# lucidrains/progen

Hardware: AMD Instinct MI355X
Metric: train tokens/sec (whole node) (higher is better)
Workload: dtype bf16; 1 GPU; model=ProGen-1.2B, global_batch=64, seq_len=1024, parallelism=dp1

## Files before the change

progen_amd/models/progen.py:

```python

from __future__ import annotations

import math
from typing import Any, Dict, Optional

import torch
import torch.nn as nn

from ..config import ProGenConfig
from ..ops import functional as OF
from ..ops import reference as R


def _haiku_linear_init_(weight: torch.Tensor, bias: Optional[torch.Tensor],
                        generator: Optional[torch.Generator] = None) -> None:
    fan_in = weight.shape[1]
    std = 1.0 / math.sqrt(fan_in)
    with torch.no_grad():
        weight.normal_(0.0, std, generator=generator).clamp_(-2 * std, 2 * std)
        if bias is not None:
            bias.zero_()


class Linear(nn.Linear):

    def reset_parameters(self) -> None:
        _haiku_linear_init_(self.weight, self.bias)

    def forward(self, x: torch.Tensor) -> torch.Tensor:
        from ..ops import fp8
        if fp8.fp8_eligible(x, self.weight):
            return fp8.fp8_linear(x, self.weight, self.bias)
        from ..ops.overlap import overlap_linear
        return overlap_linear(x, self.weight, self.bias)


class LocalAttention(nn.Module):

    def __init__(self, cfg: ProGenConfig):
        super().__init__()
        self.heads = cfg.heads
        self.window_size = cfg.window_size
        self.shift_tokens = cfg.shift_tokens
        inner = cfg.inner_dim
        self.norm_weight = nn.Parameter(torch.ones(cfg.dim))
        self.to_qkv = Linear(cfg.dim, inner * 3, bias=False)
        self.to_out = Linear(inner, cfg.dim, bias=True)

    def forward(self, x: torch.Tensor, sin: torch.Tensor, cos: torch.Tensor) -> torch.Tensor:
        x = OF.ln_shift(x, self.norm_weight, shift=self.shift_tokens)
        return self.inner(x, sin, cos)

    def inner(self, y: torch.Tensor, sin: torch.Tensor, cos: torch.Tensor) -> torch.Tensor:
        qkv = self.to_qkv(y)
        out = OF.local_attention(qkv, sin, cos, self.heads, self.window_size)
        return self.to_out(out)


class SGU(nn.Module):

    def __init__(self, dim: int, dim_out: int, seq_len: int, eps: float = 1e-3):
        super().__init__()
        self.seq_len = seq_len
        self.norm_weight = nn.Parameter(torch.ones(dim // 2))
        init_scale = eps / seq_len
        self.spatial_weights = nn.Parameter(
            torch.empty(seq_len, seq_len).uniform_(-init_scale, init_scale))
        self.spatial_biases = nn.Parameter(torch.ones(seq_len, 1))
        self.proj_out = Linear(dim // 2, dim_out, bias=True)

    def forward(self, x: torch.Tensor) -> torch.Tensor:
# ... 9 lines not shown
        assert not (glu and spatial_gate), \
            "glu and sgu cannot be turned on at the same time"
        hidden = cfg.dim * cfg.ff_mult * (2 if glu else 1)
        self.glu = glu
        self.shift_tokens = cfg.shift_tokens
        self.norm_weight = nn.Parameter(torch.ones(cfg.dim))
        self.proj_in = Linear(cfg.dim, hidden, bias=True)
        self.sgu = SGU(hidden, hidden // 2, cfg.seq_len) if spatial_gate else None
        out_in = hidden // 2 if (glu or spatial_gate) else hidden
        self.proj_out = Linear(out_in, cfg.dim, bias=True)

    def forward(self, x: torch.Tensor) -> torch.Tensor:
        x = OF.ln_shift(x, self.norm_weight, shift=self.shift_tokens)
        return self.inner(x)

    def inner(self, x: torch.Tensor) -> torch.Tensor:
        x = self.proj_in(x)
        if self.glu:
            x = OF.glu_gelu(x)
        else:
            x = OF.gelu(x)
        if self.sgu is not None:
            x = self.sgu(x)
        return self.proj_out(x)


class ProGenBase(nn.Module):

    def __init__(self, cfg: ProGenConfig):
        super().__init__()
        self.cfg = cfg
        self.embed = nn.Embedding(cfg.num_tokens, cfg.dim)
        with torch.no_grad():
            std = 1.0 / math.sqrt(cfg.num_tokens)
            self.embed.weight.normal_(0.0, std).clamp_(-2 * std, 2 * std)

        layers = []
        for i in range(cfg.depth):
            use_gmlp = (cfg.depth - i) <= cfg.global_mlp_depth
# ... 11 lines not shown
        self.register_buffer("rotary_sin", sin, persistent=False)
        self.register_buffer("rotary_cos", cos, persistent=False)

    def forward(self, x: torch.Tensor) -> torch.Tensor:
        if x.dim() == 1:
            x = x.unsqueeze(0)
        n = x.shape[1]
        if self.rotary_sin.dtype != torch.float32:
            sin, cos = R.fixed_pos_embedding(self.cfg.seq_len,
                                             self.cfg.dim_head,
                                             device=self.rotary_sin.device)
            self.rotary_sin, self.rotary_cos = sin, cos
        sin = self.rotary_sin[:n]
        cos = self.rotary_cos[:n]
        h = self.embed(x.long())
        r = None
        for attn, ff in self.layers:
            y, h = OF.ln_shift_res(h, r, attn.norm_weight,
                                   shift=attn.shift_tokens)
            a = attn.inner(y, sin, cos)
            y, h = OF.ln_shift_res(h, a, ff.norm_weight,
                                   shift=ff.shift_tokens)
            r = ff.inner(y)
        y, _ = OF.ln_shift_res(h, r, self.final_norm_weight, shift=False)
        return self.to_logits(y)

    def num_params(self) -> int:
        return sum(p.numel() for p in self.parameters())



class TransformedProGen:

    def __init__(self, cfg: ProGenConfig, module: Optional[ProGenBase] = None):
        self.cfg = cfg
        self.module = module if module is not None else ProGenBase(cfg)

    @staticmethod
    def _seed_everything(rng) -> None:
# ... 37 lines not shown
```

progen_amd/ops/functional.py:

```python

from __future__ import annotations

import torch
import torch.nn.functional as F

from . import dispatch, reference



class _LnShiftFn(torch.autograd.Function):
    @staticmethod
    def forward(ctx, x, weight, shift: bool, eps: float):
        C = dispatch.ext()
        y, mean, rstd = C.ln_shift_fwd(x, weight, bool(shift), float(eps))
        ctx.save_for_backward(x, weight, mean, rstd)
        ctx.shift = bool(shift)
        return y

    @staticmethod
    def backward(ctx, dy):
        x, weight, mean, rstd = ctx.saved_tensors
        C = dispatch.ext()
        dx, dweight = C.ln_shift_bwd(dy.contiguous(), x, weight, mean, rstd, ctx.shift)
        return dx, dweight, None, None


def ln_shift(x: torch.Tensor, weight: torch.Tensor, shift: bool = True,
             eps: float = 1e-5) -> torch.Tensor:
    if dispatch.use_hip(x, "ln"):
        return _LnShiftFn.apply(x, weight, shift, eps)
    return reference.ln_shift(x, weight, shift, eps)


class _LnShiftResFn(torch.autograd.Function):

    @staticmethod
    def forward(ctx, x, res, weight, shift: bool, eps: float):
        C = dispatch.ext()
        y, s, mean, rstd = C.ln_shift_res_fwd(x, res, weight, bool(shift),
                                              float(eps))
        ctx.save_for_backward(s, weight, mean, rstd)
        ctx.shift = bool(shift)
        ctx.set_materialize_grads(False)
        return y, s

    @staticmethod
    def backward(ctx, dy, ds):
        s, weight, mean, rstd = ctx.saved_tensors
        C = dispatch.ext()
        ds = ds.contiguous() if ds is not None else None
        dx, dweight = C.ln_shift_res_bwd(dy.contiguous(), ds, s, weight,
                                         mean, rstd, ctx.shift)
        return dx, dx, dweight, None, None


def ln_shift_res(x: torch.Tensor, res, weight: torch.Tensor,
                 shift: bool = True, eps: float = 1e-5):
    if dispatch.use_hip(x, "ln"):
        if res is None:
            return _LnShiftFn.apply(x, weight, shift, eps), x
        return _LnShiftResFn.apply(x, res.contiguous(), weight, shift, eps)
    s = x if res is None else x + res
    return reference.ln_shift(s, weight, shift, eps), s



class _LocalAttnFn(torch.autograd.Function):
    @staticmethod
    def forward(ctx, qkv, sin, cos, heads: int, window_size: int, halo):
        C = dispatch.ext()
        qkv_rot = C.rope_qkv(qkv.contiguous(), sin, cos)
        out, lse = C.attn_fwd(qkv_rot, int(heads), int(window_size),
                              halo=halo)
        ctx.save_for_backward(qkv_rot, sin, cos, out, lse,
                              *([halo] if halo is not None else []))
        ctx.heads = int(heads)
# ... 12 lines not shown
        dhalo = res[1].to(dout.dtype) if ctx.has_halo else None
        return dqkv, None, None, None, None, dhalo


def local_attention(qkv: torch.Tensor, sin: torch.Tensor, cos: torch.Tensor,
                    heads: int, window_size: int,
                    halo: torch.Tensor = None) -> torch.Tensor:
    if dispatch.use_hip(qkv, "attn"):
        return _LocalAttnFn.apply(qkv, sin, cos, heads, window_size, halo)
    assert halo is None, "halo is a kernel-path (GPU) feature"
    return reference.local_attention(qkv, sin, cos, heads, window_size)



class _GluGeluFn(torch.autograd.Function):
    @staticmethod
    def forward(ctx, h):
        C = dispatch.ext()
        y = C.glu_fwd(h)
        ctx.save_for_backward(h)
        return y

    @staticmethod
    def backward(ctx, dy):
        (h,) = ctx.saved_tensors
        C = dispatch.ext()
        return C.glu_bwd(dy.contiguous(), h)


def glu_gelu(h: torch.Tensor) -> torch.Tensor:
    if dispatch.use_hip(h, "glu"):
        return _GluGeluFn.apply(h)
    return reference.glu_gelu(h)


class _GeluFn(torch.autograd.Function):
    @staticmethod
    def forward(ctx, h):
        C = dispatch.ext()
        y = C.gelu_fwd(h)
        ctx.save_for_backward(h)
        return y

    @staticmethod
    def backward(ctx, dy):
        (h,) = ctx.saved_tensors
        C = dispatch.ext()
# ... 264 lines not shown
```

progen_amd/ops/hip/bindings.cpp:

```cpp

#include <torch/extension.h>

#include "checks.h"
#include "kernels.h"

using namespace chk;


static std::vector<at::Tensor> ln_shift_fwd_impl(const char* op,
                                                 const at::Tensor& x,
                                                 const at::Tensor* res,
                                                 const at::Tensor& g,
                                                 bool shift, double eps) {
  const bool bf = dtype_bf16_or_fp32(op, ARG(x));
  dtype_same(op, ARG(g), ARG(x));
  if (res) dtype_same(op, Arg{"res", *res}, ARG(x));
  contiguous_rank(op, ARG(x), 3);
  const int64_t B = x.size(0), N = x.size(1), D = x.size(2);
  if (res) contiguous_shape(op, Arg{"res", *res}, x.sizes());
  contiguous_numel(op, ARG(g), D);
  multiple_of(op, "D", D, 16);
  const int Di = extent_int(op, "D", D), Ni = extent_int(op, "N", N);
  const int R = extent_int(op, "B*N", B * N);
  same_gpu(op, {ARG(x), ARG(g)});
// ... 16 lines not shown
std::vector<at::Tensor> ln_shift_fwd(const at::Tensor& x, const at::Tensor& g,
                                     bool shift, double eps) {
  return ln_shift_fwd_impl("ln_shift_fwd", x, nullptr, g, shift, eps);
}

std::vector<at::Tensor> ln_shift_res_fwd(const at::Tensor& x,
                                         const at::Tensor& res,
                                         const at::Tensor& g, bool shift,
                                         double eps) {
  return ln_shift_fwd_impl("ln_shift_res_fwd", x, &res, g, shift, eps);
}

static std::vector<at::Tensor> ln_shift_bwd_impl(
    const char* op, const at::Tensor& dy, const c10::optional<at::Tensor>& ds,
    Arg xa, const at::Tensor& g, const at::Tensor& mean,
    const at::Tensor& rstd, bool shift) {
  const at::Tensor& x = xa.t;
  const bool bf = dtype_bf16_or_fp32(op, xa);
  dtype_same(op, ARG(dy), xa);
  dtype_same(op, ARG(g), xa);
  if (ds) dtype_same(op, Arg{"ds", *ds}, xa);
  dtype_is(op, ARG(mean), at::kFloat);
  dtype_is(op, ARG(rstd), at::kFloat);
  contiguous_rank(op, xa, 3);
  const int64_t B = x.size(0), N = x.size(1), D = x.size(2);
  contiguous_shape(op, ARG(dy), x.sizes());
  if (ds) contiguous_shape(op, Arg{"ds", *ds}, x.sizes());
  contiguous_numel(op, ARG(g), D);
  contiguous_numel(op, ARG(mean), B * N);
  contiguous_numel(op, ARG(rstd), B * N);
  multiple_of(op, "D", D, 16);
  const int Di = extent_int(op, "D", D), Ni = extent_int(op, "N", N);
  const int R = extent_int(op, "B*N", B * N);
  same_gpu(op, {xa, ARG(dy), ARG(g), ARG(mean), ARG(rstd)});
  if (ds) same_gpu(op, {xa, Arg{"ds", *ds}});

  DeviceScope dev(x);
  const int nblocks = std::min(R, 1024);
  auto dx = at::empty_like(x);
  auto dw_part = at::empty({nblocks, D}, x.options().dtype(at::kFloat));
  LAUNCH(op, ln_shift_bwd_launch(
                 dy.data_ptr(), ds ? ds->data_ptr() : nullptr, x.data_ptr(),
                 g.data_ptr(), mean.data_ptr<float>(), rstd.data_ptr<float>(),
                 dx.data_ptr(), dw_part.data_ptr<float>(), nblocks, R, Ni, Di,
                 shift, bf, dev.stream));
  auto dw = dw_part.sum(0).to(x.scalar_type());
  return {dx, dw};
}

std::vector<at::Tensor> ln_shift_bwd(const at::Tensor& dy, const at::Tensor& x,
                                     const at::Tensor& g,
                                     const at::Tensor& mean,
                                     const at::Tensor& rstd, bool shift) {
  return ln_shift_bwd_impl("ln_shift_bwd", dy, c10::nullopt, ARG(x), g, mean,
                           rstd, shift);
}

std::vector<at::Tensor> ln_shift_res_bwd(const at::Tensor& dy,
                                         const c10::optional<at::Tensor>& ds,
                                         const at::Tensor& s_in,
                                         const at::Tensor& g,
                                         const at::Tensor& mean,
                                         const at::Tensor& rstd, bool shift) {
  return ln_shift_bwd_impl("ln_shift_res_bwd", dy, ds, ARG(s_in), g, mean,
                           rstd, shift);
}


at::Tensor glu_fwd(const at::Tensor& h) {
  const char* op = "glu_fwd";
  const bool bf = dtype_bf16_or_fp32(op, ARG(h));
  CHK(h.dim() >= 1, op, "h", h.dim(), "must have at least 1 dim");
  contiguous(op, ARG(h));
  const int64_t H2 = h.size(-1), rows = leading_rows(h);
  multiple_of(op, "H2", H2, 16);
  const int H = extent_int(op, "H2", H2) / 2;
  extent(op, "rows", rows, INT64_MAX);
  same_gpu(op, {ARG(h)});

  DeviceScope dev(h);
  auto sizes = h.sizes().vec();
  sizes.back() = H;
  auto y = at::empty(sizes, h.options());
  LAUNCH(op, glu_fwd_launch(h.data_ptr(), y.data_ptr(), rows, H, bf,
                            dev.stream));
  return y;
}

at::Tensor glu_bwd(const at::Tensor& dy, const at::Tensor& h) {
  const char* op = "glu_bwd";
  const bool bf = dtype_bf16_or_fp32(op, ARG(h));
  dtype_same(op, ARG(dy), ARG(h));
  CHK(h.dim() >= 1, op, "h", h.dim(), "must have at least 1 dim");
  contiguous(op, ARG(h));
  const int64_t H2 = h.size(-1), rows = leading_rows(h);
  auto dy_sizes = h.sizes().vec();
  dy_sizes.back() = H2 / 2;
  contiguous_shape(op, ARG(dy), dy_sizes);
  multiple_of(op, "H2", H2, 16);
  const int H = extent_int(op, "H2", H2) / 2;
  extent(op, "rows", rows, INT64_MAX);
  same_gpu(op, {ARG(h), ARG(dy)});

  DeviceScope dev(h);
  auto dh = at::empty_like(h);
  LAUNCH(op, glu_bwd_launch(dy.data_ptr(), h.data_ptr(), dh.data_ptr(), rows,
                            H, bf, dev.stream));
  return dh;
}

at::Tensor gelu_fwd(const at::Tensor& h) {
  const char* op = "gelu_fwd";
  const bool bf = dtype_bf16_or_fp32(op, ARG(h));
  contiguous(op, ARG(h));
  multiple_of(op, "h.numel()", h.numel(), 8);
  extent(op, "h.numel()", h.numel(), INT64_MAX);
  same_gpu(op, {ARG(h)});

  DeviceScope dev(h);
  auto y = at::empty_like(h);
  LAUNCH(op, gelu_fwd_launch(h.data_ptr(), y.data_ptr(), h.numel(), bf,
                             dev.stream));
// ... 443 lines not shown
                       w.options().dtype(at::kFloat8_e4m3fn));
  LAUNCH(op, quant_e4m3_t_launch(w.data_ptr(), out.data_ptr(),
                                 scale.data_ptr<float>(), Nr, Kc, dev.stream));
  return out;
}

PYBIND11_MODULE(TORCH_EXTENSION_NAME, m) {
  m.def("sgu_fwd", &sgu_fwd, "SGU causal spatial matmul forward");
  m.def("sgu_dgate", &sgu_dgate, "SGU backward: dgate");
  m.def("sgu_dw", &sgu_dw, "SGU backward: dW");
  m.def("ln_shift_fwd", &ln_shift_fwd, "fused LN+shift forward");
  m.def("ln_shift_bwd", &ln_shift_bwd, "fused LN+shift backward");
  m.def("ln_shift_res_fwd", &ln_shift_res_fwd,
        "residual-add-fused LN+shift forward");
  m.def("ln_shift_res_bwd", &ln_shift_res_bwd,
        "residual-add-fused LN+shift backward");
  m.def("glu_fwd", &glu_fwd, "GLU-GELU forward");
  m.def("glu_bwd", &glu_bwd, "GLU-GELU backward");
  m.def("gelu_fwd", &gelu_fwd, "GELU forward");
  m.def("gelu_bwd", &gelu_bwd, "GELU backward");
  m.def("ce_fwd", &ce_fwd, "fused CE forward (nll, lse)");
  m.def("ce_bwd", &ce_bwd, "fused CE backward");
  m.def("grad_sumsq", &grad_sumsq, "sum of squares of flat grads");
  m.def("fused_adamw", &fused_adamw, "fused clip+AdamW over flat space",
        py::arg("master"), py::arg("params"), py::arg("grads"),
        py::arg("exp_avg"), py::arg("exp_avg_sq"), py::arg("chunk_starts"),
        py::arg("chunk_ends"), py::arg("chunk_decay"), py::arg("lr"),
        py::arg("b1"), py::arg("b2"), py::arg("eps"), py::arg("wd"),
        py::arg("step_dev"), py::arg("grad_scale"), py::arg("clip_coef"),
        py::arg("shard_off") = 0);
  m.def("rope_qkv", &rope_qkv, "pre-rotation of qkv (rotary on q,k,v)");
  m.def("attn_fwd", &attn_fwd, "fused local attention forward",
        py::arg("qkv_rot"), py::arg("heads"), py::arg("window"),
// ... 15 lines not shown
```

progen_amd/ops/hip/common.h:

```cpp
#pragma once

#include <hip/hip_runtime.h>
#include <hip/hip_bf16.h>

#define WAVE 64

using bf16 = __hip_bfloat16;

typedef short bf16x8 __attribute__((ext_vector_type(8)));
typedef float f32x4 __attribute__((ext_vector_type(4)));
typedef float f32x16 __attribute__((ext_vector_type(16)));

__device__ __forceinline__ float bf2f(short u) {
  union { unsigned int i; float f; } c;
  c.i = ((unsigned int)(unsigned short)u) << 16;
  return c.f;
}

__device__ __forceinline__ short f2bf(float f) {
  __hip_bfloat16 b = __float2bfloat16(f);
  return *(short*)&b;
}

__device__ __forceinline__ float wave_sum(float v) {
// ... 122 lines not shown
template <bool BF>
using vec16_t = typename vec16<BF>::type;

template <bool BF>
__device__ __forceinline__ float vget(const vec16_t<BF>& v, int j) {
  if constexpr (BF) return bf2f(v[j]);
  else return v[j];
}

template <bool BF>
__device__ __forceinline__ void vset(vec16_t<BF>& v, int j, float x) {
  if constexpr (BF) v[j] = f2bf(x);
  else v[j] = x;
}

__device__ __forceinline__ float block256_sum(float v, float* red) {
  v = wave_sum(v);
  if ((threadIdx.x & 63) == 0) red[threadIdx.x >> 6] = v;
  __syncthreads();
  return red[0] + red[1] + red[2] + red[3];
}
```

progen_amd/ops/hip/glu.hip:

```cpp

#include "common.h"

#define GLU_BLOCK 256

template <bool BF>
__global__ __launch_bounds__(GLU_BLOCK) void glu_fwd_kernel(
    const void* __restrict__ h_, void* __restrict__ y_, long long rows,
    int Hv) {
  using VEC = vec16_t<BF>;
  const VEC* h = (const VEC*)h_;
  VEC* y = (VEC*)y_;
  const int i = blockIdx.x * GLU_BLOCK + (int)threadIdx.x;
  if (i >= Hv) return;
  for (long long row = blockIdx.y; row < rows; row += gridDim.y) {
    const VEC va = h[row * 2 * Hv + i];
    const VEC vg = h[row * 2 * Hv + Hv + i];
    VEC o;
#pragma unroll
    for (int j = 0; j < vec16<BF>::N; ++j)
      vset<BF>(o, j, vget<BF>(va, j) * gelu_tanh(vget<BF>(vg, j)));
    y[row * Hv + i] = o;
  }
}

template <bool BF>
__global__ __launch_bounds__(GLU_BLOCK) void glu_bwd_kernel(
    const void* __restrict__ dy_, const void* __restrict__ h_,
    void* __restrict__ dh_, long long rows, int Hv) {
  using VEC = vec16_t<BF>;
  const VEC *dy = (const VEC*)dy_, *h = (const VEC*)h_;
  VEC* dh = (VEC*)dh_;
  const int i = blockIdx.x * GLU_BLOCK + (int)threadIdx.x;
  if (i >= Hv) return;
  for (long long row = blockIdx.y; row < rows; row += gridDim.y) {
    const VEC va = h[row * 2 * Hv + i];
    const VEC vg = h[row * 2 * Hv + Hv + i];
    const VEC vdy = dy[row * Hv + i];
    VEC da, dg;
#pragma unroll
    for (int j = 0; j < vec16<BF>::N; ++j) {
      const float d = vget<BF>(vdy, j);
      float gv, gg;
      gelu_tanh_both(vget<BF>(vg, j), &gv, &gg);
      vset<BF>(da, j, d * gv);
      vset<BF>(dg, j, d * vget<BF>(va, j) * gg);
    }
    dh[row * 2 * Hv + i] = da;
    dh[row * 2 * Hv + Hv + i] = dg;
  }
}

template <bool BF>
__global__ __launch_bounds__(GLU_BLOCK) void gelu_fwd_kernel(
    const void* __restrict__ h_, void* __restrict__ y_, long long total) {
  using VEC = vec16_t<BF>;
  const VEC* h = (const VEC*)h_;
  VEC* y = (VEC*)y_;
  for (long long idx = blockIdx.x * (long long)GLU_BLOCK + threadIdx.x;
       idx < total; idx += (long long)gridDim.x * GLU_BLOCK) {
    const VEC v = h[idx];
    VEC o;
#pragma unroll
    for (int j = 0; j < vec16<BF>::N; ++j)
// ... 86 lines not shown
```

progen_amd/ops/hip/kernels.h:

```cpp
#pragma once
#include <hip/hip_runtime.h>

extern "C" {

hipError_t ln_shift_fwd_launch(const void* x, const void* res, const void* g,
                               void* y, void* s_out, float* mean, float* rstd,
                               int R, int N, int D, float eps, bool shift,
                               bool is_bf16, hipStream_t stream);
hipError_t ln_shift_bwd_launch(const void* dy, const void* ds, const void* x,
                               const void* g, const float* mean,
                               const float* rstd, void* dx, float* dw_part,
                               int nblocks, int R, int N, int D, bool shift,
                               bool is_bf16, hipStream_t stream);

hipError_t glu_fwd_launch(const void* h, void* y, long long rows, int H,
                          bool is_bf16, hipStream_t stream);
hipError_t glu_bwd_launch(const void* dy, const void* h, void* dh,
                          long long rows, int H, bool is_bf16,
                          hipStream_t stream);
hipError_t gelu_fwd_launch(const void* h, void* y, long long total_elems,
                           bool is_bf16, hipStream_t stream);
hipError_t gelu_bwd_launch(const void* dy, const void* h, void* dh,
                           long long total_elems, bool is_bf16,
                           hipStream_t stream);

hipError_t ce_fwd_launch(const void* logits, const long long* targets,
                         float* nll, float* lse, long long R, int V,
                         bool is_bf16, hipStream_t stream);
hipError_t ce_bwd_launch(const float* dnll, const void* logits,
                         const long long* targets, const float* lse,
                         void* dlogits, long long R, int V, bool is_bf16,
                         hipStream_t stream);

hipError_t grad_sumsq_launch(const void* grads, float* out, long long numel,
                             bool is_bf16, hipStream_t stream);
hipError_t fused_adamw_launch(float* master, void* params, const void* grads,
                              float* exp_avg, float* exp_avg_sq,
                              const long long* starts, const long long* ends,
                              const int* decay_flags, int nchunks, float lr,
// ... 38 lines not shown
```

progen_amd/ops/hip/ln_shift.hip:

```cpp

#include <type_traits>

#include "common.h"

#define LN_BLOCK 256
#define LN_WAVES (LN_BLOCK / WAVE)

__device__ __forceinline__ float ln_block_sum(float a, float* red) {
  const int wid = threadIdx.x / WAVE;
  const int lane = threadIdx.x % WAVE;
  a = wave_sum(a);
  if (lane == 0) red[wid] = a;
  __syncthreads();
  if (wid == 0) {
    float t = (lane < LN_WAVES) ? red[lane] : 0.f;
#pragma unroll
    for (int off = LN_WAVES / 2; off > 0; off >>= 1) t += __shfl_xor(t, off, 64);
    if (lane == 0) red[0] = t;
  }
  __syncthreads();
  a = red[0];
  __syncthreads();
  return a;
}

__device__ __forceinline__ float mul_rn(float x, float y) {
#pragma clang fp contract(off)
  return x * y;
}


template <bool BF, bool SHIFT, bool RES>
__global__ __launch_bounds__(LN_BLOCK) void ln_shift_fwd_kernel(
    const void* __restrict__ x_, const void* __restrict__ res_,
    const void* __restrict__ g_, void* __restrict__ y_,
    void* __restrict__ s_out_, float* __restrict__ mean,
    float* __restrict__ rstd, int N, int Dv, float eps) {
  using VEC = vec16_t<BF>;
  constexpr int VLEN = vec16<BF>::N;
  const VEC *x = (const VEC*)x_, *res = (const VEC*)res_, *g = (const VEC*)g_;
  VEC *y = (VEC*)y_, *s_out = (VEC*)s_out_;
  const int row = blockIdx.x;
  const int n = row % N;
  const long long base = (long long)row * Dv;
// ... 49 lines not shown
      } else if (n + 1 < N) {
        y[base + Dv + i] = o;
      }
      if (ONE) break;
    }
  };
  if (Dv <= LN_BLOCK) body(std::true_type{});
  else body(std::false_type{});

  if (SHIFT && n == 0) {
    const VEC z = {};
    for (int i = threadIdx.x; i < halfv; i += LN_BLOCK) y[base + i] = z;
  }
}


template <bool BF, bool SHIFT, bool DS>
__global__ __launch_bounds__(LN_BLOCK) void ln_shift_bwd_kernel(
    const void* __restrict__ dy_, const void* __restrict__ ds_,
    const void* __restrict__ x_, const void* __restrict__ g_,
    const float* __restrict__ mean, const float* __restrict__ rstd,
    void* __restrict__ dx_, float* __restrict__ dw_part, int R, int N,
    int Dv) {
  using VEC = vec16_t<BF>;
  constexpr int VLEN = vec16<BF>::N;
  const VEC *dy = (const VEC*)dy_, *ds = (const VEC*)ds_;
  const VEC *x = (const VEC*)x_, *g = (const VEC*)g_;
  VEC* dx = (VEC*)dx_;
  const int D = Dv * VLEN;
  const int halfv = (D / 2) / VLEN;

  extern __shared__ __attribute__((aligned(16))) char smem[];
  float* dw_lds = (float*)smem;
  float* red = (float*)(smem + (size_t)D * 4);

  for (int i = threadIdx.x; i < D; i += LN_BLOCK) dw_lds[i] = 0.f;
  __syncthreads();

  auto rows = [&](auto one) {
    constexpr bool ONE = decltype(one)::value;
    for (int row = blockIdx.x; row < R; row += gridDim.x) {
      const int n = row % N;
      const long long base = (long long)row * Dv;
      const float mu = mean[row];
      const float rs = rstd[row];
      const float inv_d = 1.0f / D;

      VEC e, v, gw, dsv;
      auto fetch = [&](int i) {
        if (DS) dsv = ds[base + i];
        if (!SHIFT || i >= halfv) e = dy[base + i];
        else if (n + 1 < N) e = dy[base + Dv + i];
        else e = VEC{};
        v = x[base + i];
        gw = g[i];
      };

      float a = 0.f, bsum = 0.f;
      for (int i = threadIdx.x; i < Dv; i += LN_BLOCK) {
        fetch(i);
#pragma unroll
        for (int j = 0; j < VLEN; ++j) {
          const float ej = vget<BF>(e, j), gj = vget<BF>(gw, j);
          const float xh = (vget<BF>(v, j) - mu) * rs;
          const float eg = mul_rn(ej, gj);
          a += mul_rn(eg, xh);
          bsum += eg;
        }
        if (ONE) break;
      }
      a = ln_block_sum(a, red);
      bsum = ln_block_sum(bsum, red);

      for (int i = threadIdx.x; i < Dv; i += LN_BLOCK) {
        if (!ONE) fetch(i);
        VEC o;
#pragma unroll
        for (int j = 0; j < VLEN; ++j) {
          const float ej = vget<BF>(e, j), gj = vget<BF>(gw, j);
          const float xh = (vget<BF>(v, j) - mu) * rs;
          float dxv = rs * (ej * gj - bsum * inv_d - xh * a * inv_d);
          if (DS) dxv += vget<BF>(dsv, j);
          vset<BF>(o, j, dxv);
          dw_lds[i * VLEN + j] += ej * xh;
        }
        dx[base + i] = o;
        if (ONE) break;
      }
      __syncthreads();
    }
  };
  if (Dv <= LN_BLOCK) rows(std::true_type{});
  else rows(std::false_type{});

  float* out = dw_part + (size_t)blockIdx.x * D;
  for (int i = threadIdx.x; i < D; i += LN_BLOCK) out[i] = dw_lds[i];
}

#define LN_KERNEL(K, i) K<((i) & 4) != 0, ((i) & 2) != 0, ((i) & 1) != 0>
#define LN_TABLE(K)                                                     \
  {LN_KERNEL(K, 0), LN_KERNEL(K, 1), LN_KERNEL(K, 2), LN_KERNEL(K, 3), \
   LN_KERNEL(K, 4), LN_KERNEL(K, 5), LN_KERNEL(K, 6), LN_KERNEL(K, 7)}

extern "C" {

hipError_t ln_shift_fwd_launch(const void* x, const void* res, const void* g,
                               void* y, void* s_out, float* mean, float* rstd,
                               int R, int N, int D, float eps, bool shift,
                               bool is_bf16, hipStream_t stream) {
  static constexpr decltype(&ln_shift_fwd_kernel<true, true, true>)
      kernels[8] = LN_TABLE(ln_shift_fwd_kernel);
  const int Dv = D / (is_bf16 ? 8 : 4);
  const auto kernel = kernels[is_bf16 * 4 + shift * 2 + (res != nullptr)];
  kernel<<<R, LN_BLOCK, 0, stream>>>(x, res, g, y, s_out, mean, rstd, N, Dv,
                                     eps);
  return hipGetLastError();
}
// ... 18 lines not shown
```

setup.py:

```python

import glob
import os

from setuptools import setup

os.environ.setdefault("PYTORCH_ROCM_ARCH", "gfx950")

from torch.utils.cpp_extension import BuildExtension, CUDAExtension

EXTENSIONS = {
    "progen_amd._C": [
        "progen_amd/ops/hip/bindings.cpp",
        "progen_amd/ops/hip/ln_shift.hip",
        "progen_amd/ops/hip/glu.hip",
        "progen_amd/ops/hip/cross_entropy.hip",
        "progen_amd/ops/hip/adamw.hip",
        "progen_amd/ops/hip/rope_qkv.hip",
        "progen_amd/ops/hip/attention_fwd.hip",
        "progen_amd/ops/hip/attention_bwd.hip",
        "progen_amd/ops/hip/sgu.hip",
        "progen_amd/ops/hip/fp8_quant.hip",
        "progen_amd/ops/hip/colsum.hip",
    ],
    "progen_amd._C_decode": [
        "progen_amd/ops/hip/decode_bindings.cpp",
        "progen_amd/ops/hip/decode_ln_shift.hip",
        "progen_amd/ops/hip/decode_attn.hip",
        "progen_amd/ops/hip/decode_sgu.hip",
    ],
# ... 47 lines not shown
```

Measured before the change: 104,600 tokens/s.

## Fuse linear bias gradients into LayerNorm-residual and GLU backward kernels

Linear layers whose output feeds a LayerNorm-residual or GLU op now run with a detached bias. The bias gradient is then computed inside the consumer's backward kernel by reducing dx or dh column-wise through per-block partials. This removes the separate column-sum pass over the output gradient that autograd would otherwise launch for each bias. In exchange the LN and GLU backward kernels use more LDS and extra partial buffers, plus an extra sum_out reduction. The path is disabled when the fp8 or overlap linear routes are active.

```diff
diff --git a/progen_amd/models/progen.py b/progen_amd/models/progen.py
--- a/progen_amd/models/progen.py
+++ b/progen_amd/models/progen.py
@@ -6,6 +6,7 @@
 
 import torch
 import torch.nn as nn
+import torch.nn.functional as F
 
 from ..config import ProGenConfig
 from ..ops import functional as OF
@@ -35,6 +36,13 @@
         return overlap_linear(x, self.weight, self.bias)
 
 
+def linear_handing_bias_on(lin: nn.Module, x: torch.Tensor, consumer: str):
+    if type(lin) is Linear and OF.fused_dbias(x, lin.weight, lin.bias,
+                                              consumer):
+        return F.linear(x, lin.weight, lin.bias.detach()), lin.bias
+    return lin(x), None
+
+
 class LocalAttention(nn.Module):
 
     def __init__(self, cfg: ProGenConfig):
@@ -51,10 +59,18 @@
         x = OF.ln_shift(x, self.norm_weight, shift=self.shift_tokens)
         return self.inner(x, sin, cos)
 
+    def _context(self, y: torch.Tensor, sin: torch.Tensor,
+                 cos: torch.Tensor) -> torch.Tensor:
+        qkv = self.to_qkv(y)
+        return OF.local_attention(qkv, sin, cos, self.heads, self.window_size)
+
     def inner(self, y: torch.Tensor, sin: torch.Tensor, cos: torch.Tensor) -> torch.Tensor:
-        qkv = self.to_qkv(y)
-        out = OF.local_attention(qkv, sin, cos, self.heads, self.window_size)
-        return self.to_out(out)
+        return self.to_out(self._context(y, sin, cos))
+
+    def inner_with_bias(self, y: torch.Tensor, sin: torch.Tensor,
+                        cos: torch.Tensor, consumer: str):
+        return linear_handing_bias_on(self.to_out, self._context(y, sin, cos),
+                                      consumer)
 
 
 class SGU(nn.Module):
@@ -94,15 +110,21 @@
         x = OF.ln_shift(x, self.norm_weight, shift=self.shift_tokens)
         return self.inner(x)
 
-    def inner(self, x: torch.Tensor) -> torch.Tensor:
-        x = self.proj_in(x)
+    def _hidden(self, x: torch.Tensor) -> torch.Tensor:
         if self.glu:
-            x = OF.glu_gelu(x)
+            x, bias = linear_handing_bias_on(self.proj_in, x, "glu")
+            x = OF.glu_gelu(x, bias)
         else:
-            x = OF.gelu(x)
+            x = OF.gelu(self.proj_in(x))
         if self.sgu is not None:
             x = self.sgu(x)
-        return self.proj_out(x)
+        return x
+
+    def inner(self, x: torch.Tensor) -> torch.Tensor:
+        return self.proj_out(self._hidden(x))
+
+    def inner_with_bias(self, x: torch.Tensor, consumer: str):
+        return linear_handing_bias_on(self.proj_out, self._hidden(x), consumer)
 
 
 class ProGenBase(nn.Module):
@@ -144,15 +166,16 @@
         sin = self.rotary_sin[:n]
         cos = self.rotary_cos[:n]
         h = self.embed(x.long())
-        r = None
+        r = r_bias = None
         for attn, ff in self.layers:
             y, h = OF.ln_shift_res(h, r, attn.norm_weight,
-                                   shift=attn.shift_tokens)
-            a = attn.inner(y, sin, cos)
+                                   shift=attn.shift_tokens, res_bias=r_bias)
+            a, a_bias = attn.inner_with_bias(y, sin, cos, "ln")
             y, h = OF.ln_shift_res(h, a, ff.norm_weight,
-                                   shift=ff.shift_tokens)
-            r = ff.inner(y)
-        y, _ = OF.ln_shift_res(h, r, self.final_norm_weight, shift=False)
+                                   shift=ff.shift_tokens, res_bias=a_bias)
+            r, r_bias = ff.inner_with_bias(y, "ln")
+        y, _ = OF.ln_shift_res(h, r, self.final_norm_weight, shift=False,
+                               res_bias=r_bias)
         return self.to_logits(y)
 
     def num_params(self) -> int:
diff --git a/progen_amd/ops/functional.py b/progen_amd/ops/functional.py
--- a/progen_amd/ops/functional.py
+++ b/progen_amd/ops/functional.py
@@ -1,10 +1,32 @@
 
 from __future__ import annotations
+
+import os
 
 import torch
 import torch.nn.functional as F
 
 from . import dispatch, reference
+
+
+
+def fused_dbias(x: torch.Tensor, weight: torch.Tensor, bias, tag: str) -> bool:
+    if bias is None or not bias.requires_grad:
+        return False
+    if os.environ.get("PROGEN_FUSED_DBIAS", "1") == "0":
+        return False
+    if not dispatch.use_hip(x, tag):
+        return False
+    from . import fp8, overlap
+    if fp8.fp8_eligible(x, weight):
+        return False
+    return not (overlap.ENABLED or overlap.FN_LINEAR)
+
+
+def _bias_grad_buffer(bias_dtype, n: int, device):
+    if bias_dtype is None:
+        return None
+    return torch.empty(n, dtype=torch.float32, device=device)
 
 
 
@@ -35,12 +57,13 @@
 class _LnShiftResFn(torch.autograd.Function):
 
     @staticmethod
-    def forward(ctx, x, res, weight, shift: bool, eps: float):
+    def forward(ctx, x, res, weight, shift: bool, eps: float, res_bias=None):
         C = dispatch.ext()
         y, s, mean, rstd = C.ln_shift_res_fwd(x, res, weight, bool(shift),
                                               float(eps))
         ctx.save_for_backward(s, weight, mean, rstd)
         ctx.shift = bool(shift)
+        ctx.bias_dtype = None if res_bias is None else res_bias.dtype
         ctx.set_materialize_grads(False)
         return y, s
 
@@ -49,17 +72,25 @@
         s, weight, mean, rstd = ctx.saved_tensors
         C = dispatch.ext()
         ds = ds.contiguous() if ds is not None else None
+        db = _bias_grad_buffer(ctx.bias_dtype, s.shape[-1], s.device)
         dx, dweight = C.ln_shift_res_bwd(dy.contiguous(), ds, s, weight,
-                                         mean, rstd, ctx.shift)
-        return dx, dx, dweight, None, None
+                                         mean, rstd, ctx.shift, db)
+        if db is not None:
+            db = db.to(ctx.bias_dtype)
+        return dx, dx, dweight, None, None, db
 
 
 def ln_shift_res(x: torch.Tensor, res, weight: torch.Tensor,
-                 shift: bool = True, eps: float = 1e-5):
-    if dispatch.use_hip(x, "ln"):
+                 shift: bool = True, eps: float = 1e-5, res_bias=None):
+    hip = dispatch.use_hip(x, "ln")
+    if res_bias is not None and (res is None or not hip):
+        raise RuntimeError("ln_shift_res: res_bias needs the HIP kernel and a "
+                           "res to deliver its gradient (see fused_dbias)")
+    if hip:
         if res is None:
             return _LnShiftFn.apply(x, weight, shift, eps), x
-        return _LnShiftResFn.apply(x, res.contiguous(), weight, shift, eps)
+        return _LnShiftResFn.apply(x, res.contiguous(), weight, shift, eps,
+                                   res_bias)
     s = x if res is None else x + res
     return reference.ln_shift(s, weight, shift, eps), s
 
@@ -102,23 +133,33 @@
 
 
 class _GluGeluFn(torch.autograd.Function):
-    @staticmethod
-    def forward(ctx, h):
+
+    @staticmethod
+    def forward(ctx, h, bias=None):
         C = dispatch.ext()
         y = C.glu_fwd(h)
         ctx.save_for_backward(h)
+        ctx.bias_dtype = None if bias is None else bias.dtype
         return y
 
     @staticmethod
     def backward(ctx, dy):
         (h,) = ctx.saved_tensors
         C = dispatch.ext()
-        return C.glu_bwd(dy.contiguous(), h)
-
-
-def glu_gelu(h: torch.Tensor) -> torch.Tensor:
-    if dispatch.use_hip(h, "glu"):
-        return _GluGeluFn.apply(h)
+        db = _bias_grad_buffer(ctx.bias_dtype, h.shape[-1], h.device)
+        dh = C.glu_bwd(dy.contiguous(), h, db)
+        if db is not None:
+            db = db.to(ctx.bias_dtype)
+        return dh, db
+
+
+def glu_gelu(h: torch.Tensor, bias=None) -> torch.Tensor:
+    hip = dispatch.use_hip(h, "glu")
+    if bias is not None and not hip:
+        raise RuntimeError("glu_gelu: bias needs the HIP kernel to deliver "
+                           "its gradient (see fused_dbias)")
+    if hip:
+        return _GluGeluFn.apply(h, bias)
     return reference.glu_gelu(h)
 
 
diff --git a/progen_amd/ops/hip/bias_grad.hip b/progen_amd/ops/hip/bias_grad.hip
--- /dev/null
+++ b/progen_amd/ops/hip/bias_grad.hip
@@ -0,0 +1,92 @@
+
+#include "glu_bwd_body.h"
+#include "ln_shift_bwd_body.h"
+
+template <bool BF>
+__global__ __launch_bounds__(GLU_BLOCK) void glu_bwd_db_kernel(
+    const void* __restrict__ dy_, const void* __restrict__ h_,
+    void* __restrict__ dh_, float* __restrict__ part, long long rows,
+    int Hv) {
+  using VEC = vec16_t<BF>;
+  constexpr int VLEN = vec16<BF>::N;
+  const VEC *dy = (const VEC*)dy_, *h = (const VEC*)h_;
+  VEC* dh = (VEC*)dh_;
+  const int i = blockIdx.x * GLU_BLOCK + (int)threadIdx.x;
+  if (i >= Hv) return;
+  float sa[VLEN], sg[VLEN];
+#pragma unroll
+  for (int j = 0; j < VLEN; ++j) sa[j] = sg[j] = 0.f;
+  for (long long row = blockIdx.y; row < rows; row += gridDim.y) {
+    VEC da, dg;
+    glu_bwd_row<BF>(dy, h, dh, row, Hv, i, da, dg);
+    opaque_vec(da);
+    opaque_vec(dg);
+#pragma unroll
+    for (int j = 0; j < VLEN; ++j) {
+      sa[j] += vget<BF>(da, j);
+      sg[j] += vget<BF>(dg, j);
+    }
+  }
+  f32x4* out = (f32x4*)(part + (size_t)blockIdx.y * 2 * Hv * VLEN);
+#pragma unroll
+  for (int q = 0; q < VLEN / 4; ++q) {
+    out[i * (VLEN / 4) + q] =
+        f32x4{sa[4 * q], sa[4 * q + 1], sa[4 * q + 2], sa[4 * q + 3]};
+    out[(Hv + i) * (VLEN / 4) + q] =
+        f32x4{sg[4 * q], sg[4 * q + 1], sg[4 * q + 2], sg[4 * q + 3]};
+  }
+}
+
+template <bool BF, bool SHIFT, bool DS>
+__global__ __launch_bounds__(LN_BLOCK) void ln_shift_bwd_db_kernel(
+    const void* __restrict__ dy_, const void* __restrict__ ds_,
+    const void* __restrict__ x_, const void* __restrict__ g_,
+    const float* __restrict__ mean, const float* __restrict__ rstd,
+    void* __restrict__ dx_, float* __restrict__ dw_part,
+    float* __restrict__ db_part, int R, int N, int Dv) {
+  ln_shift_bwd_body<BF, SHIFT, DS, true>(dy_, ds_, x_, g_, mean, rstd, dx_,
+                                         dw_part, db_part, R, N, Dv);
+}
+
+extern "C" {
+
+int glu_bwd_db_stripes(long long rows, int H, bool is_bf16) {
+  const int Hv = H / (is_bf16 ? 8 : 4);
+  const int gx = (Hv + GLU_BLOCK - 1) / GLU_BLOCK;
+  long long gy = 1024 / gx;
+  if (gy < 1) gy = 1;
+  if (gy > rows) gy = rows;
+  return (int)gy;
+}
+
+hipError_t glu_bwd_db_launch(const void* dy, const void* h, void* dh,
+                             float* part, int stripes, long long rows, int H,
+                             bool is_bf16, hipStream_t stream) {
+  const int Hv = H / (is_bf16 ? 8 : 4);
+  const dim3 grid((Hv + GLU_BLOCK - 1) / GLU_BLOCK, (unsigned)stripes);
+  if (is_bf16)
+    glu_bwd_db_kernel<true><<<grid, GLU_BLOCK, 0, stream>>>(dy, h, dh, part,
+                                                            rows, Hv);
+  else
+    glu_bwd_db_kernel<false><<<grid, GLU_BLOCK, 0, stream>>>(dy, h, dh, part,
+                                                             rows, Hv);
+  return hipGetLastError();
+}
+
+hipError_t ln_shift_bwd_db_launch(const void* dy, const void* ds,
+                                  const void* x, const void* g,
+                                  const float* mean, const float* rstd,
+                                  void* dx, float* dw_part, float* db_part,
+                                  int nblocks, int R, int N, int D, bool shift,
+                                  bool is_bf16, hipStream_t stream) {
+  static constexpr decltype(&ln_shift_bwd_db_kernel<true, true, true>)
+      kernels[8] = LN_TABLE(ln_shift_bwd_db_kernel);
+  const int Dv = D / (is_bf16 ? 8 : 4);
+  const size_t lds = (size_t)D * 8 + LN_WAVES * 4 + 16;
+  const auto kernel = kernels[is_bf16 * 4 + shift * 2 + (ds != nullptr)];
+  kernel<<<nblocks, LN_BLOCK, lds, stream>>>(dy, ds, x, g, mean, rstd, dx,
+                                             dw_part, db_part, R, N, Dv);
+  return hipGetLastError();
+}
+
+}
diff --git a/progen_amd/ops/hip/bindings.cpp b/progen_amd/ops/hip/bindings.cpp
--- a/progen_amd/ops/hip/bindings.cpp
+++ b/progen_amd/ops/hip/bindings.cpp
@@ -54,7 +54,8 @@
 static std::vector<at::Tensor> ln_shift_bwd_impl(
     const char* op, const at::Tensor& dy, const c10::optional<at::Tensor>& ds,
     Arg xa, const at::Tensor& g, const at::Tensor& mean,
-    const at::Tensor& rstd, bool shift) {
+    const at::Tensor& rstd, bool shift,
+    const c10::optional<at::Tensor>& db) {
   const at::Tensor& x = xa.t;
   const bool bf = dtype_bf16_or_fp32(op, xa);
   dtype_same(op, ARG(dy), xa);
@@ -62,6 +63,7 @@
   if (ds) dtype_same(op, Arg{"ds", *ds}, xa);
   dtype_is(op, ARG(mean), at::kFloat);
   dtype_is(op, ARG(rstd), at::kFloat);
+  if (db) dtype_is(op, Arg{"db", *db}, at::kFloat);
   contiguous_rank(op, xa, 3);
   const int64_t B = x.size(0), N = x.size(1), D = x.size(2);
   contiguous_shape(op, ARG(dy), x.sizes());
@@ -69,21 +71,36 @@
   contiguous_numel(op, ARG(g), D);
   contiguous_numel(op, ARG(mean), B * N);
   contiguous_numel(op, ARG(rstd), B * N);
+  if (db) contiguous_shape(op, Arg{"db", *db}, {D});
   multiple_of(op, "D", D, 16);
   const int Di = extent_int(op, "D", D), Ni = extent_int(op, "N", N);
   const int R = extent_int(op, "B*N", B * N);
   same_gpu(op, {xa, ARG(dy), ARG(g), ARG(mean), ARG(rstd)});
   if (ds) same_gpu(op, {xa, Arg{"ds", *ds}});
+  if (db) same_gpu(op, {xa, Arg{"db", *db}});
 
   DeviceScope dev(x);
   const int nblocks = std::min(R, 1024);
   auto dx = at::empty_like(x);
   auto dw_part = at::empty({nblocks, D}, x.options().dtype(at::kFloat));
-  LAUNCH(op, ln_shift_bwd_launch(
-                 dy.data_ptr(), ds ? ds->data_ptr() : nullptr, x.data_ptr(),
-                 g.data_ptr(), mean.data_ptr<float>(), rstd.data_ptr<float>(),
-                 dx.data_ptr(), dw_part.data_ptr<float>(), nblocks, R, Ni, Di,
-                 shift, bf, dev.stream));
+  if (db) {
+    auto db_part = at::empty_like(dw_part);
+    LAUNCH(op, ln_shift_bwd_db_launch(
+                   dy.data_ptr(), ds ? ds->data_ptr() : nullptr, x.data_ptr(),
+                   g.data_ptr(), mean.data_ptr<float>(),
+                   rstd.data_ptr<float>(), dx.data_ptr(),
+                   dw_part.data_ptr<float>(), db_part.data_ptr<float>(),
+                   nblocks, R, Ni, Di, shift, bf, dev.stream));
+    at::Tensor db_out = *db;
+    at::sum_out(db_out, db_part, {0});
+  } else {
+    LAUNCH(op, ln_shift_bwd_launch(
+                   dy.data_ptr(), ds ? ds->data_ptr() : nullptr, x.data_ptr(),
+                   g.data_ptr(), mean.data_ptr<float>(),
+                   rstd.data_ptr<float>(), dx.data_ptr(),
+                   dw_part.data_ptr<float>(), nblocks, R, Ni, Di, shift, bf,
+                   dev.stream));
+  }
   auto dw = dw_part.sum(0).to(x.scalar_type());
   return {dx, dw};
 }
@@ -93,7 +110,7 @@
                                      const at::Tensor& mean,
                                      const at::Tensor& rstd, bool shift) {
   return ln_shift_bwd_impl("ln_shift_bwd", dy, c10::nullopt, ARG(x), g, mean,
-                           rstd, shift);
+                           rstd, shift, c10::nullopt);
 }
 
 std::vector<at::Tensor> ln_shift_res_bwd(const at::Tensor& dy,
@@ -101,9 +118,10 @@
                                          const at::Tensor& s_in,
                                          const at::Tensor& g,
                                          const at::Tensor& mean,
-                                         const at::Tensor& rstd, bool shift) {
+                                         const at::Tensor& rstd, bool shift,
+                                         const c10::optional<at::Tensor>& db) {
   return ln_shift_bwd_impl("ln_shift_res_bwd", dy, ds, ARG(s_in), g, mean,
-                           rstd, shift);
+                           rstd, shift, db);
 }
 
 
@@ -127,25 +145,39 @@
   return y;
 }
 
-at::Tensor glu_bwd(const at::Tensor& dy, const at::Tensor& h) {
+at::Tensor glu_bwd(const at::Tensor& dy, const at::Tensor& h,
+                   const c10::optional<at::Tensor>& db) {
   const char* op = "glu_bwd";
   const bool bf = dtype_bf16_or_fp32(op, ARG(h));
   dtype_same(op, ARG(dy), ARG(h));
+  if (db) dtype_is(op, Arg{"db", *db}, at::kFloat);
   CHK(h.dim() >= 1, op, "h", h.dim(), "must have at least 1 dim");
   contiguous(op, ARG(h));
   const int64_t H2 = h.size(-1), rows = leading_rows(h);
   auto dy_sizes = h.sizes().vec();
   dy_sizes.back() = H2 / 2;
   contiguous_shape(op, ARG(dy), dy_sizes);
+  if (db) contiguous_shape(op, Arg{"db", *db}, {H2});
   multiple_of(op, "H2", H2, 16);
   const int H = extent_int(op, "H2", H2) / 2;
   extent(op, "rows", rows, INT64_MAX);
   same_gpu(op, {ARG(h), ARG(dy)});
+  if (db) same_gpu(op, {ARG(h), Arg{"db", *db}});
 
   DeviceScope dev(h);
   auto dh = at::empty_like(h);
-  LAUNCH(op, glu_bwd_launch(dy.data_ptr(), h.data_ptr(), dh.data_ptr(), rows,
-                            H, bf, dev.stream));
+  if (db) {
+    const int stripes = glu_bwd_db_stripes(rows, H, bf);
+    auto part = at::empty({stripes, H2}, h.options().dtype(at::kFloat));
+    LAUNCH(op, glu_bwd_db_launch(dy.data_ptr(), h.data_ptr(), dh.data_ptr(),
+                                 part.data_ptr<float>(), stripes, rows, H, bf,
+                                 dev.stream));
+    at::Tensor db_out = *db;
+    at::sum_out(db_out, part, {0});
+  } else {
+    LAUNCH(op, glu_bwd_launch(dy.data_ptr(), h.data_ptr(), dh.data_ptr(), rows,
+                              H, bf, dev.stream));
+  }
   return dh;
 }
 
@@ -619,9 +651,14 @@
   m.def("ln_shift_res_fwd", &ln_shift_res_fwd,
         "residual-add-fused LN+shift forward");
   m.def("ln_shift_res_bwd", &ln_shift_res_bwd,
-        "residual-add-fused LN+shift backward");
+        "residual-add-fused LN+shift backward; db: also the column sums of dx",
+        py::arg("dy"), py::arg("ds"), py::arg("s_in"), py::arg("g"),
+        py::arg("mean"), py::arg("rstd"), py::arg("shift"),
+        py::arg("db") = py::none());
   m.def("glu_fwd", &glu_fwd, "GLU-GELU forward");
-  m.def("glu_bwd", &glu_bwd, "GLU-GELU backward");
+  m.def("glu_bwd", &glu_bwd,
+        "GLU-GELU backward; db: also the column sums of dh", py::arg("dy"),
+        py::arg("h"), py::arg("db") = py::none());
   m.def("gelu_fwd", &gelu_fwd, "GELU forward");
   m.def("gelu_bwd", &gelu_bwd, "GELU backward");
   m.def("ce_fwd", &ce_fwd, "fused CE forward (nll, lse)");
diff --git a/progen_amd/ops/hip/common.h b/progen_amd/ops/hip/common.h
--- a/progen_amd/ops/hip/common.h
+++ b/progen_amd/ops/hip/common.h
@@ -160,6 +160,11 @@
   else v[j] = x;
 }
 
+template <typename VEC>
+__device__ __forceinline__ void opaque_vec(VEC& v) {
+  asm volatile("" : "+v"(v));
+}
+
 __device__ __forceinline__ float block256_sum(float v, float* red) {
   v = wave_sum(v);
   if ((threadIdx.x & 63) == 0) red[threadIdx.x >> 6] = v;
diff --git a/progen_amd/ops/hip/glu.hip b/progen_amd/ops/hip/glu.hip
--- a/progen_amd/ops/hip/glu.hip
+++ b/progen_amd/ops/hip/glu.hip
@@ -1,7 +1,6 @@
 
 #include "common.h"
-
-#define GLU_BLOCK 256
+#include "glu_bwd_body.h"
 
 template <bool BF>
 __global__ __launch_bounds__(GLU_BLOCK) void glu_fwd_kernel(
@@ -33,20 +32,8 @@
   const int i = blockIdx.x * GLU_BLOCK + (int)threadIdx.x;
   if (i >= Hv) return;
   for (long long row = blockIdx.y; row < rows; row += gridDim.y) {
-    const VEC va = h[row * 2 * Hv + i];
-    const VEC vg = h[row * 2 * Hv + Hv + i];
-    const VEC vdy = dy[row * Hv + i];
     VEC da, dg;
-#pragma unroll
-    for (int j = 0; j < vec16<BF>::N; ++j) {
-      const float d = vget<BF>(vdy, j);
-      float gv, gg;
-      gelu_tanh_both(vget<BF>(vg, j), &gv, &gg);
-      vset<BF>(da, j, d * gv);
-      vset<BF>(dg, j, d * vget<BF>(va, j) * gg);
-    }
-    dh[row * 2 * Hv + i] = da;
-    dh[row * 2 * Hv + Hv + i] = dg;
+    glu_bwd_row<BF>(dy, h, dh, row, Hv, i, da, dg);
   }
 }
 
diff --git a/progen_amd/ops/hip/glu_bwd_body.h b/progen_amd/ops/hip/glu_bwd_body.h
--- /dev/null
+++ b/progen_amd/ops/hip/glu_bwd_body.h
@@ -0,0 +1,31 @@
+#pragma once
+
+#include "common.h"
+
+#define GLU_BLOCK 256
+
+template <bool BF>
+__device__ __forceinline__ void glu_bwd_row(const vec16_t<BF>* dy,
+                                            const vec16_t<BF>* h,
+                                            vec16_t<BF>* dh, long long row,
+                                            int Hv, int i,
+                                            vec16_t<BF>& da_out,
+                                            vec16_t<BF>& dg_out) {
+  using VEC = vec16_t<BF>;
+  const VEC va = h[row * 2 * Hv + i];
+  const VEC vg = h[row * 2 * Hv + Hv + i];
+  const VEC vdy = dy[row * Hv + i];
+  VEC da, dg;
+#pragma unroll
+  for (int j = 0; j < vec16<BF>::N; ++j) {
+    const float d = vget<BF>(vdy, j);
+    float gv, gg;
+    gelu_tanh_both(vget<BF>(vg, j), &gv, &gg);
+    vset<BF>(da, j, d * gv);
+    vset<BF>(dg, j, d * vget<BF>(va, j) * gg);
+  }
+  dh[row * 2 * Hv + i] = da;
+  dh[row * 2 * Hv + Hv + i] = dg;
+  da_out = da;
+  dg_out = dg;
+}
diff --git a/progen_amd/ops/hip/kernels.h b/progen_amd/ops/hip/kernels.h
--- a/progen_amd/ops/hip/kernels.h
+++ b/progen_amd/ops/hip/kernels.h
@@ -23,6 +23,17 @@
 hipError_t gelu_bwd_launch(const void* dy, const void* h, void* dh,
                            long long total_elems, bool is_bf16,
                            hipStream_t stream);
+
+int glu_bwd_db_stripes(long long rows, int H, bool is_bf16);
+hipError_t glu_bwd_db_launch(const void* dy, const void* h, void* dh,
+                             float* part, int stripes, long long rows, int H,
+                             bool is_bf16, hipStream_t stream);
+hipError_t ln_shift_bwd_db_launch(const void* dy, const void* ds,
+                                  const void* x, const void* g,
+                                  const float* mean, const float* rstd,
+                                  void* dx, float* dw_part, float* db_part,
+                                  int nblocks, int R, int N, int D, bool shift,
+                                  bool is_bf16, hipStream_t stream);
 
 hipError_t ce_fwd_launch(const void* logits, const long long* targets,
                          float* nll, float* lse, long long R, int V,
diff --git a/progen_amd/ops/hip/ln_common.h b/progen_amd/ops/hip/ln_common.h
--- /dev/null
+++ b/progen_amd/ops/hip/ln_common.h
@@ -0,0 +1,29 @@
+#pragma once
+
+#include "common.h"
+
+#define LN_BLOCK 256
+#define LN_WAVES (LN_BLOCK / WAVE)
+
+#define LN_KERNEL(K, i) K<((i) & 4) != 0, ((i) & 2) != 0, ((i) & 1) != 0>
+#define LN_TABLE(K)                                                     \
+  {LN_KERNEL(K, 0), LN_KERNEL(K, 1), LN_KERNEL(K, 2), LN_KERNEL(K, 3), \
+   LN_KERNEL(K, 4), LN_KERNEL(K, 5), LN_KERNEL(K, 6), LN_KERNEL(K, 7)}
+
+__device__ __forceinline__ float ln_block_sum(float a, float* red) {
+  const int wid = threadIdx.x / WAVE;
+  const int lane = threadIdx.x % WAVE;
+  a = wave_sum(a);
+  if (lane == 0) red[wid] = a;
+  __syncthreads();
+  if (wid == 0) {
+    float t = (lane < LN_WAVES) ? red[lane] : 0.f;
+#pragma unroll
+    for (int off = LN_WAVES / 2; off > 0; off >>= 1) t += __shfl_xor(t, off, 64);
+    if (lane == 0) red[0] = t;
+  }
+  __syncthreads();
+  a = red[0];
+  __syncthreads();
+  return a;
+}
diff --git a/progen_amd/ops/hip/ln_shift.hip b/progen_amd/ops/hip/ln_shift.hip
--- a/progen_amd/ops/hip/ln_shift.hip
+++ b/progen_amd/ops/hip/ln_shift.hip
@@ -1,33 +1,8 @@
 
 #include <type_traits>
 
-#include "common.h"
-
-#define LN_BLOCK 256
-#define LN_WAVES (LN_BLOCK / WAVE)
-
-__device__ __forceinline__ float ln_block_sum(float a, float* red) {
-  const int wid = threadIdx.x / WAVE;
-  const int lane = threadIdx.x % WAVE;
-  a = wave_sum(a);
-  if (lane == 0) red[wid] = a;
-  __syncthreads();
-  if (wid == 0) {
-    float t = (lane < LN_WAVES) ? red[lane] : 0.f;
-#pragma unroll
-    for (int off = LN_WAVES / 2; off > 0; off >>= 1) t += __shfl_xor(t, off, 64);
-    if (lane == 0) red[0] = t;
-  }
-  __syncthreads();
-  a = red[0];
-  __syncthreads();
-  return a;
-}
-
-__device__ __forceinline__ float mul_rn(float x, float y) {
-#pragma clang fp contract(off)
-  return x * y;
-}
+#include "ln_common.h"
+#include "ln_shift_bwd_body.h"
 
 
 template <bool BF, bool SHIFT, bool RES>
@@ -107,7 +82,6 @@
   }
 }
 
-
 template <bool BF, bool SHIFT, bool DS>
 __global__ __launch_bounds__(LN_BLOCK) void ln_shift_bwd_kernel(
     const void* __restrict__ dy_, const void* __restrict__ ds_,
@@ -115,85 +89,10 @@
     const float* __restrict__ mean, const float* __restrict__ rstd,
     void* __restrict__ dx_, float* __restrict__ dw_part, int R, int N,
     int Dv) {
-  using VEC = vec16_t<BF>;
-  constexpr int VLEN = vec16<BF>::N;
-  const VEC *dy = (const VEC*)dy_, *ds = (const VEC*)ds_;
-  const VEC *x = (const VEC*)x_, *g = (const VEC*)g_;
-  VEC* dx = (VEC*)dx_;
-  const int D = Dv * VLEN;
-  const int halfv = (D / 2) / VLEN;
-
-  extern __shared__ __attribute__((aligned(16))) char smem[];
-  float* dw_lds = (float*)smem;
-  float* red = (float*)(smem + (size_t)D * 4);
-
-  for (int i = threadIdx.x; i < D; i += LN_BLOCK) dw_lds[i] = 0.f;
-  __syncthreads();
-
-  auto rows = [&](auto one) {
-    constexpr bool ONE = decltype(one)::value;
-    for (int row = blockIdx.x; row < R; row += gridDim.x) {
-      const int n = row % N;
-      const long long base = (long long)row * Dv;
-      const float mu = mean[row];
-      const float rs = rstd[row];
-      const float inv_d = 1.0f / D;
-
-      VEC e, v, gw, dsv;
-      auto fetch = [&](int i) {
-        if (DS) dsv = ds[base + i];
-        if (!SHIFT || i >= halfv) e = dy[base + i];
-        else if (n + 1 < N) e = dy[base + Dv + i];
-        else e = VEC{};
-        v = x[base + i];
-        gw = g[i];
-      };
-
-      float a = 0.f, bsum = 0.f;
-      for (int i = threadIdx.x; i < Dv; i += LN_BLOCK) {
-        fetch(i);
-#pragma unroll
-        for (int j = 0; j < VLEN; ++j) {
-          const float ej = vget<BF>(e, j), gj = vget<BF>(gw, j);
-          const float xh = (vget<BF>(v, j) - mu) * rs;
-          const float eg = mul_rn(ej, gj);
-          a += mul_rn(eg, xh);
-          bsum += eg;
-        }
-        if (ONE) break;
-      }
-      a = ln_block_sum(a, red);
-      bsum = ln_block_sum(bsum, red);
-
-      for (int i = threadIdx.x; i < Dv; i += LN_BLOCK) {
-        if (!ONE) fetch(i);
-        VEC o;
-#pragma unroll
-        for (int j = 0; j < VLEN; ++j) {
-          const float ej = vget<BF>(e, j), gj = vget<BF>(gw, j);
-          const float xh = (vget<BF>(v, j) - mu) * rs;
-          float dxv = rs * (ej * gj - bsum * inv_d - xh * a * inv_d);
-          if (DS) dxv += vget<BF>(dsv, j);
-          vset<BF>(o, j, dxv);
-          dw_lds[i * VLEN + j] += ej * xh;
-        }
-        dx[base + i] = o;
-        if (ONE) break;
-      }
-      __syncthreads();
-    }
-  };
-  if (Dv <= LN_BLOCK) rows(std::true_type{});
-  else rows(std::false_type{});
-
-  float* out = dw_part + (size_t)blockIdx.x * D;
-  for (int i = threadIdx.x; i < D; i += LN_BLOCK) out[i] = dw_lds[i];
+  ln_shift_bwd_body<BF, SHIFT, DS, false>(dy_, ds_, x_, g_, mean, rstd, dx_,
+                                          dw_part, nullptr, R, N, Dv);
 }
 
-#define LN_KERNEL(K, i) K<((i) & 4) != 0, ((i) & 2) != 0, ((i) & 1) != 0>
-#define LN_TABLE(K)                                                     \
-  {LN_KERNEL(K, 0), LN_KERNEL(K, 1), LN_KERNEL(K, 2), LN_KERNEL(K, 3), \
-   LN_KERNEL(K, 4), LN_KERNEL(K, 5), LN_KERNEL(K, 6), LN_KERNEL(K, 7)}
 
 extern "C" {
 
diff --git a/progen_amd/ops/hip/ln_shift_bwd_body.h b/progen_amd/ops/hip/ln_shift_bwd_body.h
--- /dev/null
+++ b/progen_amd/ops/hip/ln_shift_bwd_body.h
@@ -0,0 +1,106 @@
+#pragma once
+
+#include <type_traits>
+
+#include "ln_common.h"
+
+__device__ __forceinline__ float mul_rn(float x, float y) {
+#pragma clang fp contract(off)
+  return x * y;
+}
+
+template <bool BF, bool SHIFT, bool DS, bool DB>
+__device__ __forceinline__ void ln_shift_bwd_body(
+    const void* __restrict__ dy_, const void* __restrict__ ds_,
+    const void* __restrict__ x_, const void* __restrict__ g_,
+    const float* __restrict__ mean, const float* __restrict__ rstd,
+    void* __restrict__ dx_, float* __restrict__ dw_part,
+    float* __restrict__ db_part, int R, int N, int Dv) {
+  using VEC = vec16_t<BF>;
+  constexpr int VLEN = vec16<BF>::N;
+  const VEC *dy = (const VEC*)dy_, *ds = (const VEC*)ds_;
+  const VEC *x = (const VEC*)x_, *g = (const VEC*)g_;
+  VEC* dx = (VEC*)dx_;
+  const int D = Dv * VLEN;
+  const int halfv = (D / 2) / VLEN;
+
+  extern __shared__ __attribute__((aligned(16))) char smem[];
+  float* dw_lds = (float*)smem;
+  float* db_lds = dw_lds + D;
+  float* red = (float*)(smem + (size_t)D * 4 * (DB ? 2 : 1));
+
+  for (int i = threadIdx.x; i < D; i += LN_BLOCK) {
+    dw_lds[i] = 0.f;
+    if (DB) db_lds[i] = 0.f;
+  }
+  __syncthreads();
+
+  auto rows = [&](auto one) {
+    constexpr bool ONE = decltype(one)::value;
+    for (int row = blockIdx.x; row < R; row += gridDim.x) {
+      const int n = row % N;
+      const long long base = (long long)row * Dv;
+      const float mu = mean[row];
+      const float rs = rstd[row];
+      const float inv_d = 1.0f / D;
+
+      VEC e, v, gw, dsv;
+      auto fetch = [&](int i) {
+        if (DS) dsv = ds[base + i];
+        if (!SHIFT || i >= halfv) e = dy[base + i];
+        else if (n + 1 < N) e = dy[base + Dv + i];
+        else e = VEC{};
+        v = x[base + i];
+        gw = g[i];
+      };
+
+      float a = 0.f, bsum = 0.f;
+      for (int i = threadIdx.x; i < Dv; i += LN_BLOCK) {
+        fetch(i);
+#pragma unroll
+        for (int j = 0; j < VLEN; ++j) {
+          const float ej = vget<BF>(e, j), gj = vget<BF>(gw, j);
+          const float xh = (vget<BF>(v, j) - mu) * rs;
+          const float eg = mul_rn(ej, gj);
+          a += mul_rn(eg, xh);
+          bsum += eg;
+        }
+        if (ONE) break;
+      }
+      a = ln_block_sum(a, red);
+      bsum = ln_block_sum(bsum, red);
+
+      for (int i = threadIdx.x; i < Dv; i += LN_BLOCK) {
+        if (!ONE) fetch(i);
+        VEC o;
+#pragma unroll
+        for (int j = 0; j < VLEN; ++j) {
+          const float ej = vget<BF>(e, j), gj = vget<BF>(gw, j);
+          const float xh = (vget<BF>(v, j) - mu) * rs;
+          float dxv = rs * (ej * gj - bsum * inv_d - xh * a * inv_d);
+          if (DS) dxv += vget<BF>(dsv, j);
+          vset<BF>(o, j, dxv);
+          dw_lds[i * VLEN + j] += ej * xh;
+        }
+        dx[base + i] = o;
+        if (DB) {
+          opaque_vec(o);
+#pragma unroll
+          for (int j = 0; j < VLEN; ++j)
+            db_lds[i * VLEN + j] += vget<BF>(o, j);
+        }
+        if (ONE) break;
+      }
+      __syncthreads();
+    }
+  };
+  if (Dv <= LN_BLOCK) rows(std::true_type{});
+  else rows(std::false_type{});
+
+  float* out = dw_part + (size_t)blockIdx.x * D;
+  for (int i = threadIdx.x; i < D; i += LN_BLOCK) out[i] = dw_lds[i];
+  if (DB) {
+    float* bout = db_part + (size_t)blockIdx.x * D;
+    for (int i = threadIdx.x; i < D; i += LN_BLOCK) bout[i] = db_lds[i];
+  }
+}
diff --git a/setup.py b/setup.py
--- a/setup.py
+++ b/setup.py
@@ -13,6 +13,7 @@
         "progen_amd/ops/hip/bindings.cpp",
         "progen_amd/ops/hip/ln_shift.hip",
         "progen_amd/ops/hip/glu.hip",
+        "progen_amd/ops/hip/bias_grad.hip",
         "progen_amd/ops/hip/cross_entropy.hip",
         "progen_amd/ops/hip/adamw.hip",
         "progen_amd/ops/hip/rope_qkv.hip",
```

Measured after the change: 106,400 tokens/s, median of 6. +1.8%, better.
